# davdwan21/Silent-Speech

Hardware: AMD Instinct MI355X
Metric: clips/sec (30-frame, fwd+bwd) (higher is better)
Workload: dtype f32; 1 GPU; BASELINE config 2: landmark (K=40, D=84) + 64x64 uint8 ROI CNN + 2-layer BiGRU(192), T=30, C=5, train step = fwd + CE(ls .05) + bwd + grad all-reduce + clip(1.0) + Adam, dropout on; batch_per_gpu=256, global_batch=256, frames=30, parallelism=dp1, micro_batches_in_flight=1

## Files before the change

### include/ss_hotpath.h

```cpp
#ifndef SS_HOTPATH_H
#define SS_HOTPATH_H

#include <stdint.h>

#ifdef __cplusplus
extern "C" {
#endif

typedef void* ss_stream_t;

enum ss_status {
  SS_OK = 0,
  SS_ERR_ARG = -1,
  SS_ERR_LAUNCH = -2,
  SS_ERR_UNSUPPORTED = -3
};

int ss_abi_version(void);
const char* ss_status_string(int status);

int ss_feature_fuse(const float* lm, const uint8_t* reset, int B, int T, int K, int w, int h, int a_left,
                    int a_right, int a_up, int a_lo, int variant, float* X, int ldx, float* center,
                    double* fourth, ss_stream_t stream);

// ... 34 lines not shown
int ss_roi_cnn_bwd(const uint8_t* R, int N, int H, int W, int standardize, const float* w1, const float* b1,
                   const float* w2, const float* b2, const float* w3, const float* b3, const float* wfc,
                   const float* bfc, int E, const float* st_a1, const uint8_t* st_i1, const float* st_a2,
                   const uint8_t* st_i2, const uint8_t* st_m3, const float* st_feat, const int* stash_sizes,
                   const float* d_out, int ld_dout, float* g_w1, float* g_b1, float* g_w2, float* g_b2, float* g_w3, float* g_b3,
                   float* g_wfc, float* g_bfc, ss_stream_t stream);

int ss_roi_active_frames(const int32_t* lengths, int B, int T, int* frames, float* emb, int ld_emb, int emb_cols,
                         ss_stream_t stream);
int ss_roi_cnn_fwd_frames(const uint8_t* R, int N, int H, int W, int standardize, const float* w1, const float* b1,
                          const float* w2, const float* b2, const float* w3, const float* b3, const float* wfc,
                          const float* bfc, int E, float* out, int ld_out, float* st_a1, uint8_t* st_i1,
                          float* st_a2, uint8_t* st_i2, uint8_t* st_m3, float* st_feat, const int* stash_sizes,
                          const int* frames, ss_stream_t stream);
int ss_roi_cnn_bwd_frames(const uint8_t* R, int N, int H, int W, int standardize, const float* w1, const float* b1,
                          const float* w2, const float* b2, const float* w3, const float* b3, const float* wfc,
                          const float* bfc, int E, const float* st_a1, const uint8_t* st_i1, const float* st_a2,
                          const uint8_t* st_i2, const uint8_t* st_m3, const float* st_feat, const int* stash_sizes,
                          const float* d_out, int ld_dout, float* g_w1, float* g_b1, float* g_w2, float* g_b2, float* g_w3,
                          float* g_b3, float* g_wfc, float* g_bfc, const int* frames, ss_stream_t stream);

int ss_gemm_f32(int a_kcontig, int b_kcontig, int M, int N, int K, const float* A, int lda, int a_group,
                int a_gstride, int a_off, const float* B, int ldb, int b_group, int b_gstride, int b_off,
                float* C, int ldc, const float* bias, float* a_colsum, int flags, int splits, ss_stream_t stream);

int ss_gemm_f32_batched(int a_kcontig, int b_kcontig, int M, int N, int K, const float* A, int lda, int a_group,
                        int a_gstride, int a_off, const float* B, int ldb, int b_group, int b_gstride, int b_off,
                        float* C, int ldc, const float* bias, float* a_colsum, int flags, int splits, int batch,
                        long stride_a, long stride_b, long stride_c, long stride_bias, long stride_colsum,
                        ss_stream_t stream);

int ss_gemm_splitk_ws_floats(int M, int N, int K, int splits, int batch, long* floats);
int ss_gemm_splitk_reduce(const float* ws, int M, int N, int K, int splits, int batch, float* C, int ldc, long stride_c,
                          ss_stream_t stream);

int ss_train_prologue(float* grads, long n_grads, float* scalars, int n_scalars, int32_t* correct,
                      const int64_t* lengths64, int32_t* lengths32, int B, const float* X, int ld_x, float* Z, int ld_z,
                      int rows, int cols, int* frames, int emb_cols, ss_stream_t stream);

typedef struct ss_gemm_problem {
  int a_kcontig, b_kcontig, M, N, K;
  const float* A;
  int lda, a_group, a_gstride, a_off;
  const float* B;
  int ldb, b_group, b_gstride, b_off;
  float* C;
  int ldc, splits, batch;
  long stride_a, stride_b, stride_c;
} ss_gemm_problem;
int ss_gemm_splitk_group_ws_floats(const ss_gemm_problem* problems, int n, long* floats);
int ss_gemm_f32_splitk_group(const ss_gemm_problem* problems, int n, float* ws, long ws_floats, int flags, ss_stream_t stream);
int ss_gemm_bf16_splitk_group_ws_floats(const ss_gemm_problem* problems, int n, long* floats);
int ss_gemm_bf16_splitk_group(const ss_gemm_problem* problems, int n, float* ws, long ws_floats, ss_stream_t stream);

int ss_zero_f32x2(float* a, long na, float* b, long nb, ss_stream_t stream);

int ss_colsum_f32(const float* A, int rows, int cols, int lda, float* out, ss_stream_t stream);

int ss_batch_gather_f32(const float* src, int D, const int32_t* frame_map, long rows, const float* noise,
                        const int32_t* noise_map, float noise_std, uint64_t seed, float* dst, ss_stream_t stream);
int ss_batch_gather_f32_at(const float* src, int D, const int32_t* frame_map, long rows, const int32_t* noise_map, float noise_std,
                           uint64_t seed, uint64_t noise_first, float* dst, ss_stream_t stream);
int ss_batch_gather_u8(const uint8_t* src, int frame_bytes, const int32_t* frame_map, long rows, uint8_t* dst,
                       ss_stream_t stream);
int ss_epoch_sample(const int32_t* members, int n_members, const int32_t* class_start, int n_classes, uint64_t first, long count,
                    uint64_t seed, int32_t* indices, ss_stream_t stream);
int ss_batch_plan(const int32_t* indices, int B, const int32_t* x_off, const int32_t* x_len, const int32_t* r_off,
                  const int32_t* r_len, const int64_t* y, int n_clips, int max_t, int augment, uint64_t first_row, uint64_t seed,
                  double noise_prob, double drop_prob, int drop_max, int32_t* xmap, int32_t* nmap, int32_t* rmap, int64_t* lens,
                  int64_t* y_out, int32_t* err_flag, ss_stream_t stream);
int ss_batch_plan_aug(const int32_t* indices, int B, const int32_t* x_off, const int32_t* x_len, const int32_t* r_off,
                      const int32_t* r_len, const int64_t* y, int n_clips, int max_t, int augment, uint64_t first_row, uint64_t seed,
                      double noise_prob, double drop_prob, int drop_max, double warp_prob, int warp_lo_pm, int warp_hi_pm,
                      double scale_prob, float scale_lo, float scale_span, double shift_prob, int shift_max_x, int shift_max_y,
                      int32_t* xmap, int32_t* nmap, int32_t* rmap, int64_t* lens, int64_t* y_out, float* row_scale,
                      int32_t* row_shift, int32_t* err_flag, ss_stream_t stream);
int ss_batch_gather_f32_aug(const float* src, int D, const int32_t* frame_map, long rows, const int32_t* noise_map, float noise_std,
                            uint64_t seed, uint64_t noise_first, const float* row_scale, int rows_per_clip, float* dst,
                            ss_stream_t stream);
int ss_batch_gather_u8_shift(const uint8_t* src, int H, int W, const int32_t* frame_map, long rows, const int32_t* row_shift,
                             int rows_per_clip, int shift_max_x, int shift_max_y, uint8_t* dst, ss_stream_t stream);
int ss_batch_gather_z(const float* feat, int D, const int32_t* xmap, const float* emb, int E, const int32_t* rmap,
                      const float* emb_fill, long rows, const int32_t* noise_map, float noise_std, uint64_t seed,
                      uint64_t noise_first, const float* row_scale, int rows_per_clip, float* dst, int ld_dst, ss_stream_t stream);
int ss_batch_plan_mask(int32_t* xmap, int32_t* nmap, int32_t* rmap, const int64_t* lens, int B, int max_t, int D, int H, int W,
                       int augment, uint64_t first_row, uint64_t seed, double time_mask_prob, int time_mask_max,
                       int time_mask_streams, int time_mask_fill, double feat_mask_prob, int feat_mask_max, double cutout_prob,
                       int cut_max_w, int cut_max_h, int cutout_fill, int32_t* row_mask, ss_stream_t stream);
int ss_batch_mask_apply(float* X, int ld_x, int D, uint8_t* R, int H, int W, const int32_t* rmap, const int32_t* row_mask,
                        long rows, int rows_per_clip, int fill, ss_stream_t stream);

int ss_ring_push(float* ring_x, uint8_t* ring_r, int n_streams, int max_t, int D, int frame_bytes,
                 const int32_t* stream_ids, int n, const float* feats, const uint8_t* rois, int32_t* head, int32_t* count,
                 int32_t* frames_seen, ss_stream_t stream);
int ss_ring_tick(const int32_t* stream_ids, int n, int32_t* frames_seen, ss_stream_t stream);
int ss_ring_window_map(const int32_t* stream_ids, int n, int max_t, const int32_t* head, const int32_t* count,
                       int32_t* frame_map, int64_t* lengths, ss_stream_t stream);
int ss_mouth_openness(const float* lm, int n, int K, int mode, int i_top, int i_bot, int i_eye_l, int i_eye_r,
                      double* openness, ss_stream_t stream);
int ss_mouth_gate(const int32_t* stream_ids, int n, const double* openness, double alpha, double open_thr,
                  double close_thr, double* ema, uint8_t* state_open, ss_stream_t stream);
int ss_clip_gate(const int32_t* stream_ids, int n, const double* openv, const uint8_t* face_present, double open_thresh,
                 int start_n, int end_n, int max_clip, int min_clip, int32_t* state, int D, int frame_bytes,
                 const float* feats, const uint8_t* rois, float* clip_x, uint8_t* clip_r, int32_t* append_row,
                 int32_t* emit_len, ss_stream_t stream);

// ... 139 lines not shown
```

### silent_speech_amd/_lib.py

```python
from __future__ import annotations

import ctypes as C
import os

import torch

_HERE = os.path.dirname(os.path.abspath(__file__))
LIB_PATH = os.environ.get("SS_HOTPATH_LIB", os.path.join(_HERE, "libss_hotpath.so"))

_vp = C.c_void_p
_i = C.c_int
_f = C.c_float
_l = C.c_long
_u64 = C.c_uint64
_d = C.c_double

SIGNATURES = {
    "ss_abi_version": [],
    "ss_status_string": [_i],
    "ss_feature_fuse": [_vp, _vp, _i, _i, _i, _i, _i, _i, _i, _i, _i, _i, _vp, _i, _vp, _vp, _vp],
    "ss_feature_fuse_stream": [_vp, _vp, _vp, _i, _i, _i, _i, _i, _i, _i, _i, _i, _i, _d, _d, _vp, _vp, _vp, _i, _vp, _vp, _vp, _vp],
    "ss_roi_norm": [_vp, _i, _i, _i, _vp, _vp, _vp],
    "ss_im2col3x3": [_vp, _i, _i, _i, _i, _vp, _i, _vp],
    "ss_relu_pool2": [_vp, _i, _i, _i, _i, _vp, _vp, _vp],
    "ss_relu_mean": [_vp, _i, _i, _i, _vp, _vp, _vp],
    "ss_mask_scale": [_vp, _vp, _i, _i, _i, _vp, _vp],
    "ss_col2im3x3": [_vp, _i, _i, _i, _i, _i, _vp, _vp],
    "ss_pool2_bwd": [_vp, _vp, _vp, _i, _i, _i, _i, _vp, _vp],
    "ss_roi_crop_idx": [_vp, _vp, _i, _i, _i, _i, _vp, _vp],
    "ss_roi_cnn_fwd": [_vp, _i, _i, _i, _i] + [_vp] * 8 + [_i, _vp, _i, _vp],
    "ss_roi_cnn_fwd_stash": [_vp, _i, _i, _i, _i] + [_vp] * 8 + [_i, _vp, _i] + [_vp] * 6 + [_vp, _vp],
    "ss_roi_cnn_set_max_workgroups": [_i],
    "ss_roi_active_frames": [_vp, _i, _i, _vp, _vp, _i, _i, _vp],
    "ss_roi_cnn_fwd_frames": [_vp, _i, _i, _i, _i] + [_vp] * 8 + [_i, _vp, _i] + [_vp] * 6 + [_vp, _vp, _vp],
    "ss_roi_cnn_bwd_frames": [_vp, _i, _i, _i, _i] + [_vp] * 8 + [_i] + [_vp] * 6 + [_vp, _vp, _i] + [_vp] * 8 + [_vp, _vp],
    "ss_roi_cnn_stash_size": [_i, _i, _vp],
    "ss_roi_cnn_bwd": [_vp, _i, _i, _i, _i] + [_vp] * 8 + [_i] + [_vp] * 6 + [_vp, _vp, _i] + [_vp] * 8 + [_vp],
    "ss_gemm_f32": [_i, _i, _i, _i, _i, _vp, _i, _i, _i, _i, _vp, _i, _i, _i, _i, _vp, _i, _vp, _vp, _i, _i, _vp],
    "ss_gemm_f32_batched": [_i, _i, _i, _i, _i, _vp, _i, _i, _i, _i, _vp, _i, _i, _i, _i, _vp, _i, _vp, _vp, _i, _i, _i,
                            _l, _l, _l, _l, _l, _vp],
    "ss_gemm_bf16_batched": [_i, _i, _i, _i, _i, _vp, _i, _i, _i, _i, _vp, _i, _i, _i, _i, _vp, _i, _vp, _i, _i, _i, _l, _l, _l, _l,
                             _vp],
    "ss_c5_conv1_fwd": [_vp, _i, _i, _vp, _vp, _vp, _vp, _vp, _vp],
    "ss_c5_conv_fwd": [_i, _vp, _i, _vp, _vp, _vp, _vp, _vp],
    "ss_c5_conv_last_fwd": [_vp, _i, _vp, _vp, _vp, _vp, _i, _vp, _i, _vp, _vp, _vp],
    "ss_c5_conv_wgrad": [_i, _vp, _vp, _vp, _i, _vp, _vp, _vp],
    "ss_c5_conv_dgrad": [_i, _vp, _vp, _i, _vp, _vp, _vp],
    "ss_c5_conv_last_wgrad": [_vp, _vp, _i, _i, _vp, _vp, _vp, _i, _vp, _vp, _vp, _vp, _vp],
    "ss_c5_conv_last_dgrad": [_vp, _i, _i, _vp, _vp, _i, _vp, _vp, _vp],
    "ss_c5_conv1_wgrad": [_vp, _i, _i, _vp, _vp, _vp, _vp, _vp, _vp, _vp, _vp],
    "ss_c5_conv2_dgrad_conv1_wgrad": [_vp, _vp, _i, _vp, _vp, _vp, _i, _vp, _vp, _vp, _vp, _vp, _vp],
    "ss_c5_conv12_fwd": [_vp, _i, _i, _vp, _vp, _vp, _vp, _vp, _vp, _vp, _vp],
    "ss_c5_conv_last_fwd_feat": [_vp, _i, _vp, _vp, _vp, _vp, _vp],
    "ss_c5_conv_last_wgrad_df": [_vp, _vp, _vp, _i, _vp, _vp, _vp, _l, _vp],
    "ss_c5_conv_wgrad_ws": [_i, _vp, _vp, _vp, _i, _vp, _vp, _vp, _l, _vp],
    "ss_c5_conv2_wgrad_rc_ws": [_vp, _vp, _i, _vp, _vp, _vp, _vp, _i, _vp, _vp, _vp, _l, _vp],
    "ss_c5_conv_last_dgrad_df": [_vp, _vp, _i, _vp, _vp, _vp],
    "ss_c5_conv12_fwd_i1": [_vp, _i, _i, _vp, _vp, _vp, _vp, _vp, _vp, _vp, _vp, _vp],
    "ss_c5_conv2_dgrad_conv1_wgrad_i1": [_vp, _vp, _i, _vp, _vp, _vp, _i, _vp, _vp, _vp, _vp, _vp, _vp, _vp],
    "ss_c5_conv2_wgrad_rc": [_vp, _vp, _i, _vp, _vp, _vp, _vp, _i, _vp, _vp, _vp],
    "ss_gru_bf16_prep": [_vp, _vp, _i, _vp, _vp, _vp, _vp, _i, _vp, _vp],
    "ss_gru_bf16_ws_bytes": [_i, _i, _vp],
    "ss_gru_bf16_sync_bytes": [_i, _i, _i, _vp],
    "ss_gru_bf16_fwd": [_vp, _vp, _vp, _vp, _vp, _i, _i, _i, _vp, _vp, _vp, _vp, _f, _u64, _u64, _vp, _vp, _l, _vp],
    "ss_gru_bf16_bwd": [_vp, _vp, _vp, _vp, _vp, _i, _i, _i, _vp, _vp, _f, _u64, _u64, _vp, _vp, _vp, _vp, _vp, _vp, _l, _vp],
    "ss_cvt_bf16_rows": [_vp, _i, _vp, _i, _l, _i, _f, _u64, _u64, _vp],
    "ss_gemm_splitk_ws_floats": [_i, _i, _i, _i, _i, _vp],
    "ss_gemm_splitk_reduce": [_vp, _i, _i, _i, _i, _i, _vp, _i, _l, _vp],
    "ss_gemm_splitk_group_ws_floats": [_vp, _i, _vp],
    "ss_gemm_f32_splitk_group": [_vp, _i, _vp, _l, _i, _vp],
    "ss_gemm_bf16_splitk_group_ws_floats": [_vp, _i, _vp],
    "ss_gemm_bf16_splitk_group": [_vp, _i, _vp, _l, _vp],
    "ss_colsum_f32": [_vp, _i, _i, _i, _vp, _vp],
    "ss_zero_f32x2": [_vp, _l, _vp, _l, _vp],
    "ss_train_prologue": [_vp, _l, _vp, _i, _vp, _vp, _vp, _i, _vp, _i, _vp, _i, _i, _i, _vp, _i, _vp],
    "ss_batch_gather_f32": [_vp, _i, _vp, _l, _vp, _vp, _f, _u64, _vp, _vp],
    "ss_batch_gather_f32_at": [_vp, _i, _vp, _l, _vp, _f, _u64, _u64, _vp, _vp],
    "ss_batch_gather_u8": [_vp, _i, _vp, _l, _vp, _vp],
    "ss_epoch_sample": [_vp, _i, _vp, _i, _u64, _l, _u64, _vp, _vp],
    "ss_batch_plan": [_vp, _i, _vp, _vp, _vp, _vp, _vp, _i, _i, _i, _u64, _u64, _d, _d, _i, _vp, _vp, _vp, _vp, _vp, _vp, _vp],
    "ss_batch_plan_aug": [_vp, _i, _vp, _vp, _vp, _vp, _vp, _i, _i, _i, _u64, _u64, _d, _d, _i, _d, _i, _i, _d, _f, _f, _d, _i, _i,
                          _vp, _vp, _vp, _vp, _vp, _vp, _vp, _vp, _vp],
    "ss_batch_gather_f32_aug": [_vp, _i, _vp, _l, _vp, _f, _u64, _u64, _vp, _i, _vp, _vp],
    "ss_batch_gather_u8_shift": [_vp, _i, _i, _vp, _l, _vp, _i, _i, _i, _vp, _vp],
    "ss_batch_gather_z": [_vp, _i, _vp, _vp, _i, _vp, _vp, _l, _vp, _f, _u64, _u64, _vp, _i, _vp, _i, _vp],
    "ss_batch_plan_mask": [_vp, _vp, _vp, _vp, _i, _i, _i, _i, _i, _i, _u64, _u64, _d, _i, _i, _i, _d, _i, _d, _i, _i, _i, _vp, _vp],
    "ss_batch_mask_apply": [_vp, _i, _i, _vp, _i, _i, _vp, _vp, _l, _i, _i, _vp],
    "ss_crop_gray_resize": [_vp, _i, _i, _i, _vp, _i, _i, _i, _vp, _vp],
    "ss_ring_tick": [_vp, _i, _vp, _vp],
    "ss_ring_push": [_vp, _vp, _i, _i, _i, _i, _vp, _i, _vp, _vp, _vp, _vp, _vp, _vp],
    "ss_ring_window_map": [_vp, _i, _i, _vp, _vp, _vp, _vp, _vp],
    "ss_mouth_openness": [_vp, _i, _i, _i, _i, _i, _i, _i, _vp, _vp],
    "ss_mouth_gate": [_vp, _i, _vp, _d, _d, _d, _vp, _vp, _vp],
    "ss_clip_gate": [_vp, _i, _vp, _vp, _d, _i, _i, _i, _i, _vp, _i, _i, _vp, _vp, _vp, _vp, _vp, _vp, _vp],
    "ss_gru_fwd": [_vp, _vp, _vp, _vp, _vp, _vp, _i, _i, _i, _vp, _vp, _vp, _vp],
    "ss_gru_fwd_drop": [_vp, _vp, _vp, _vp, _vp, _vp, _i, _i, _i, _vp, _vp, _vp, _f, _u64, _u64, _vp, _vp],
    "ss_gru_sync_bytes": [_i, _i, _i, _vp],
    "ss_gru_bwd": [_vp, _vp, _vp, _vp, _vp, _vp, _i, _i, _i, _vp, _f, _u64, _u64, _vp, _vp, _vp, _vp, _vp, _vp],
    "ss_gru_bias_grad": [_vp, _i, _i, _vp, _vp, _vp, _vp, _vp],
    "ss_attn_pool_fwd": [_vp, _vp, _vp, _vp, _i, _i, _i, _vp, _vp, _vp],
    "ss_attn_pool_bwd": [_vp, _vp, _vp, _vp, _vp, _i, _i, _i, _vp, _vp, _vp, _vp],
    "ss_tail_fwd": [_vp] * 11 + [_i] * 5 + [_f, _f, _u64, _u64, _f, _f] + [_vp] * 10 + [_vp],
    "ss_tail_fwd_w": [_vp] * 11 + [_i] * 5 + [_f, _f, _u64, _u64, _f, _vp, _vp] + [_vp] * 10 + [_vp],
    "ss_tail_bwd": [_vp] * 11 + [_i] * 5 + [_f, _u64, _u64] + [_vp] * 7 + [_vp],
    "ss_layernorm_fwd": [_vp, _vp, _vp, _i, _i, _f, _vp, _vp, _vp, _vp],
    "ss_layernorm_bwd": [_vp, _vp, _vp, _vp, _i, _i, _vp, _vp, _vp, _vp],
    "ss_dropout": [_vp, _vp, _l, _f, _u64, _u64, _vp, _vp],
    "ss_ce_ls_fwd_bwd": [_vp, _vp, _i, _i, _f, _f, _vp, _vp, _vp, _vp],
    "ss_eval_accum": [_vp, _vp, _i, _i, _f, _i, _vp, _vp, _vp, _vp, _vp, _vp, _vp, _vp],
    "ss_ce_ls_w_fwd_bwd": [_vp, _vp, _i, _i, _f, _vp, _vp, _vp, _vp, _vp, _vp],
    "ss_class_weight_sum": [_vp, _l, _vp, _i, _vp, _vp],
    "ss_eval_accum_w": [_vp, _vp, _i, _i, _f, _i, _vp, _vp, _vp, _vp, _vp, _vp, _vp, _vp, _vp, _vp],
    "ss_softmax_topk": [_vp, _i, _i, _i, _vp, _vp, _vp],
    "ss_sumsq_f32": [_vp, _l, _vp, _vp],
    "ss_adam_clip": [_vp, _vp, _vp, _vp, _l, _vp, _f, _f, _f, _f, _f, _f, _i, _vp],
    "ss_adam_clip_ema": [_vp, _vp, _vp, _vp, _vp, _l, _vp, _f, _f, _f, _f, _f, _f, _i, _f, _vp],
    "ss_swap_f32": [_vp, _vp, _l, _vp],
    "ss_copy_rows_f32": [_vp, _i, _vp, _i, _i, _i, _vp],
}
_RESTYPES = {"ss_status_string": C.c_char_p}

_lib = None


def load():
# ... 106 lines not shown
```

### silent_speech_amd/csrc/gemm.hip

```cpp
#include <stdlib.h>

#include <type_traits>

#define SS_STAMP_ROW ((int)(blockIdx.x + gridDim.x * (blockIdx.y + gridDim.y * blockIdx.z)))
#include "ss_common.h"

STAMP_TABLE(ss_debug_stamps_gemm)

namespace {

constexpr int BM = 128, BN = 64, BK = 16;
constexpr int LDK = BK + 4;
constexpr int LDM_A = BM + 4;
constexpr int LDM_B = BN + 4;

struct RowMap {
  int G, S, off;
  __device__ __forceinline__ long operator()(int r) const {
    if (G == 0x7fffffff) return r + off;
    return (long)(r / G) * S + (r % G) + off;
  }
};

struct GemmParams {
// ... 808 lines not shown
    for (int mt = 0; mt < 3; ++mt) a[mt] = *reinterpret_cast<const f32x4*>(st + offA[mt]);
#pragma unroll
    for (int nt = 0; nt < 6; ++nt) b[nt] = *reinterpret_cast<const f32x4*>(st + offB[nt]);
  };
  auto mma = [&]() {
#pragma unroll
    for (int kk = 0; kk < 4; ++kk)
#pragma unroll
      for (int mt = 0; mt < 3; ++mt)
#pragma unroll
        for (int nt = 0; nt < 6; ++nt) acc[mt][nt] = mfma16(a[mt][kk], b[nt][kk], acc[mt][nt]);
  };
  ring_k_loop<W_LPW>(
      nfull, rem, issue,
      [&](int stage, int refill) {
        if (refill >= 0) issue(refill);
        read(dlds + stage * W_STAGE);
        mma();
      },
      [&](int kvalid) { dp.tail(dlds, kvalid); });
  constexpr int LDS_C = 96 + 4;
  static_assert(WT * LDS_C <= DSTAGES * W_STAGE, "half an output tile is staged in the k-tile ring");
  float* Cb = P.C + bi * P.sC;
  const float* bias = P.bias ? P.bias + bi * P.sBias : nullptr;
  const bool vec_ok = (P.ldc & 3) == 0 && (reinterpret_cast<uintptr_t>(Cb) & 15) == 0;
#pragma unroll 1
  for (int h = 0; h < 2; ++h) {
    __syncthreads();
    if (wn == h) {
#pragma unroll
      for (int mt = 0; mt < 3; ++mt)
#pragma unroll
        for (int nt = 0; nt < 6; ++nt) {
          const int col = nt * 16 + i, gc = n0 + h * 96 + col;
          const float bv = (bias && gc < P.N) ? bias[gc] : 0.f;
#pragma unroll
          for (int r = 0; r < 4; ++r) dlds[(wm * 48 + mt * 16 + 4 * g + r) * LDS_C + col] = acc[mt][nt][r] + bv;
        }
    }
    __syncthreads();
    for (int q = threadIdx.x; q < WT * 24; q += WNT) {
      const int row = q / 24, c4 = 4 * (q % 24);
      const int gr = m0 + row, gc = n0 + h * 96 + c4;
      if (gr < P.M && gc < P.N) {
        const f32x4 v = *reinterpret_cast<const f32x4*>(&dlds[row * LDS_C + c4]);
        float* dst = Cb + (long)gr * P.ldc + gc;
        if (vec_ok && gc + 4 <= P.N) *reinterpret_cast<f32x4*>(dst) = v;
        else
          for (int e = 0; e < 4; ++e)
            if (gc + e < P.N) dst[e] = v[e];
      }
    }
  }
}
}

int splitk_slices(int K, int splits, int* per_out) {
  const int per = ceil_div(ceil_div(K, splits), BK * KSUB) * BK * KSUB;
  if (per_out) *per_out = per;
  return ceil_div(K, per);
}

long splitk_slab_floats(int M, int N, int K, int splits, int batch) {
  return (long)batch * splitk_slices(K, splits, nullptr) * ceil_div(M, BM) * ceil_div(N, BN) * BM * BN;
}

bool al16(const void* q) { return (reinterpret_cast<uintptr_t>(q) & 15) == 0; }

constexpr size_t dma_lds = (size_t)DSTAGES * D_STAGE * sizeof(float);
constexpr size_t wide_lds = (size_t)DSTAGES * wide::W_STAGE * sizeof(float);

template <class F>
void by_layout(bool a_kcontig, bool b_kcontig, F&& f) {
  using T = std::true_type;
  using N = std::false_type;
  if (a_kcontig && b_kcontig) f(T{}, T{});
  else if (a_kcontig && !b_kcontig) f(T{}, N{});
  else if (!a_kcontig && b_kcontig) f(N{}, T{});
  else f(N{}, N{});
}

}

extern "C" int ss_gemm_splitk_ws_floats(int M, int N, int K, int splits, int batch, long* floats) {
  SS_REQUIRE(M > 0 && N > 0 && K > 0 && splits >= 1 && batch >= 1 && floats, SS_ERR_ARG);
  *floats = splitk_slab_floats(M, N, K, splits, batch);
  return SS_OK;
}

extern "C" int ss_gemm_splitk_reduce(const float* ws, int M, int N, int K, int splits, int batch, float* C, int ldc,
                                     long stride_c, ss_stream_t stream) {
  SS_REQUIRE(ws && C && M > 0 && N > 0 && K > 0 && splits >= 1 && batch >= 1 && ldc >= N, SS_ERR_ARG);
  SS_REQUIRE((reinterpret_cast<uintptr_t>(ws) & 15) == 0, SS_ERR_ARG);
  const int nz = splitk_slices(K, splits, nullptr), gx = ceil_div(N, BN), gy = ceil_div(M, BM);
  const ReduceItem r{reinterpret_cast<const f32x4*>(ws), nz, gx, gy, M, N, C, ldc, stride_c};
  hipLaunchKernelGGL(splitk_reduce_kernel, dim3((unsigned)(batch * gx * gy * 8)), dim3(256), 0, static_cast<hipStream_t>(stream), r);
  return ss_launch_status();
}

struct GemmExtras {
  const float* bias;
  float* a_colsum;
  int flags;
  long stride_bias, stride_colsum;
};
struct GemmLaunch {
// ... 188 lines not shown
    }
  }
  GemmGroup gg;
  ReduceGroup rg;
  gg.n = rg.n = n;
  gg.first[0] = rg.first[0] = 0;
  bool grouped = true;
  for (int j = 0; j < n; ++j) {
    const ss_gemm_problem& q = problems[j];
    const ss_gemm_problem slab = group_slab_gemm(problems, j, ws);
    GemmLaunch gl;
    const int st = gemm_prepare(slab, kSlabGemm, &gl);
    if (st != SS_OK) return st;
    SS_REQUIRE(q.C && q.ldc >= q.N, SS_ERR_ARG);
    grouped = grouped && gl.dma_ok && q.a_kcontig == problems[0].a_kcontig && q.b_kcontig == problems[0].b_kcontig;
    gg.p[j] = gl.p;
    gg.gx[j] = gl.grid.x; gg.gy[j] = gl.grid.y;
    gg.first[j + 1] = gg.first[j] + (int)(gl.grid.x * gl.grid.y * gl.grid.z);
    rg.it[j] = ReduceItem{reinterpret_cast<const f32x4*>(slab.C), gl.p.nz, (int)gl.grid.x, (int)gl.grid.y, q.M, q.N, q.C, q.ldc, q.stride_c};
    rg.first[j + 1] = rg.first[j] + (int)(q.batch * gl.grid.x * gl.grid.y * 8);
  }
  for (int j = n; j < GEMM_GROUP_MAX; ++j) {
    gg.p[j] = gg.p[0]; gg.gx[j] = gg.gy[j] = 1; gg.first[j + 1] = gg.first[n];
    rg.it[j] = rg.it[0]; rg.first[j + 1] = rg.first[n];
  }
  hipStream_t s = static_cast<hipStream_t>(stream);
  if (!grouped) {
    for (int j = 0; j < n; ++j) {
      const ss_gemm_problem& q = problems[j];
      const ss_gemm_problem slab = group_slab_gemm(problems, j, ws);
      int st = gemm_batched(slab, kSlabGemm, stream);
      if (st != SS_OK) return st;
      st = ss_gemm_splitk_reduce(slab.C, q.M, q.N, q.K, q.splits, q.batch, q.C, q.ldc, q.stride_c, stream);
      if (st != SS_OK) return st;
    }
    return SS_OK;
  }
  const dim3 ggrid((unsigned)gg.first[n]), block(256);
  by_layout(problems[0].a_kcontig, problems[0].b_kcontig, [&](auto a, auto b) {
    hipLaunchKernelGGL((gemm_dma_group_kernel<decltype(a)::value, decltype(b)::value>), ggrid, block, dma_lds, s, gg);
  });
  if (ss_launch_status() != SS_OK) return SS_ERR_LAUNCH;
  hipLaunchKernelGGL(splitk_reduce_group_kernel, dim3((unsigned)rg.first[n]), dim3(256), 0, s, rg);
  return ss_launch_status();
}

extern "C" int ss_gemm_f32(int a_kcontig, int b_kcontig, int M, int N, int K, const float* A, int lda, int a_group,
                           int a_gstride, int a_off, const float* B, int ldb, int b_group, int b_gstride, int b_off,
                           float* C, int ldc, const float* bias, float* a_colsum, int flags, int splits,
                           ss_stream_t stream) {
  return ss_gemm_f32_batched(a_kcontig, b_kcontig, M, N, K, A, lda, a_group, a_gstride, a_off, B, ldb, b_group,
                             b_gstride, b_off, C, ldc, bias, a_colsum, flags, splits, 1, 0, 0, 0, 0, 0, stream);
}
```

### silent_speech_amd/engine.py

```python
from __future__ import annotations

import os

from dataclasses import dataclass
from typing import Dict, Optional

import torch

from . import _lib as L

INT_MAX = 2**31 - 1
_HH_TARGET = 512
USE_SIDE_STREAM = True


@dataclass
class Config:
    x_dim: int
    num_classes: int
    use_roi: bool
    roi_emb: int = 32
    hidden: int = 192
    gru_layers: int = 2
    roi_standardize: bool = True
    gru_dropout: float = 0.1
    head_dropout: float = 0.2
    head_mid: int = 128
    ln_eps: float = 1e-5
    cnn_channels: tuple = (8, 16, 24)
    precision: str = "f32"

    @property
    def in_dim(self) -> int:
        return self.x_dim + (self.roi_emb if self.use_roi else 0)


def gemm(a_kc, b_kc, M, N, K, A, lda, B, ldb, Cm, ldc, bias=None, accumulate=False, relu=False, splits=1,
         a_map=(INT_MAX, 0, 0), b_map=(INT_MAX, 0, 0), a_colsum=None, tag="gemm", batch=1, strides=(0, 0, 0, 0, 0),
         atomic=False, splitk_ws: Optional[torch.Tensor] = None, sum_batch=False):
    if splitk_ws is not None and splits > 1 and accumulate and not relu and bias is None:
        need = L.gemm_splitk_ws_floats(M, N, K, splits, batch)
        if splitk_ws.numel() < need:
            raise RuntimeError(f"split-K workspace too small: {splitk_ws.numel()} < {need}")
        L.call("ss_gemm_f32_batched", int(a_kc), int(b_kc), M, N, K, A, lda, a_map[0], a_map[1], a_map[2], B, ldb,
               b_map[0], b_map[1], b_map[2], splitk_ws.data_ptr(), N, None, a_colsum, 8, splits, batch,
               strides[0], strides[1], 0, 0, strides[4], L.stream(), tag=tag)
        L.call("ss_gemm_splitk_reduce", splitk_ws.data_ptr(), M, N, K, splits, batch, Cm, ldc, strides[2], L.stream(),
               tag=tag + "_reduce")
        return
    flags = (1 if accumulate else 0) | (2 if relu else 0) | (4 if atomic else 0) | (16 if sum_batch else 0)
    L.call("ss_gemm_f32_batched", int(a_kc), int(b_kc), M, N, K, A, lda, a_map[0], a_map[1], a_map[2], B, ldb,
           b_map[0], b_map[1], b_map[2], Cm, ldc, bias, a_colsum, flags, splits, batch, *strides, L.stream(), tag=tag)


_SPLITK_TARGET = 768
DW_WIDE_ALONE = 1
SKIP_PADDED_FRAMES = os.environ.get("SS_CNN_SKIP_PADDING", "1") != "0"

_DX_SPLIT_CAP = 2


def split_k(M, N, K, batch=1, target_wgs=_SPLITK_TARGET):
    tiles = -(-M // 128) * -(-N // 64) * batch
    return max(1, min(K // 128, target_wgs // tiles))


def dw_shapes(cfg, B, T, l):
    H, N = cfg.hidden, B * T
    K = cfg.in_dim if l == 0 else 2 * H
    out = [(3 * H, K, N, split_k(3 * H, K, N, 2))]
    if T > 1:
        Kh = B * (T - 1)
        out += [(2 * H, H, Kh, split_k(2 * H, H, Kh, 2, _HH_TARGET)), (H, H, Kh, split_k(H, H, Kh, 2, _HH_TARGET))]
    return out


def dw_records(cfg, B, T, l, esize, ld_in, dg, lin, hp, g_ih, g_hh, splits=None):
    H, N = cfg.hidden, B * T
    shapes = dw_shapes(cfg, B, T, l)
    splits = splits or [sh[3] for sh in shapes]
    K = shapes[0][1]

    def rec(shape, A, a_map, B_, ldb, b_map, Cm, ldc, sp, sa, sb, sc):
        return L.GemmProblem(0, 0, *shape[:3], A, 4 * H, *a_map, B_, ldb, *b_map, Cm, ldc, sp, 2, sa, sb, sc)

    ident = (INT_MAX, 0, 0)
    out = [rec(shapes[0], dg, ident, lin, ld_in, ident, g_ih[0], K, splits[0], N * 4 * H, 0, g_ih[1])]
    if T > 1:
        am, bm = (T - 1, T, 1), (T - 1, T, 0)
        sa, sb = N * 4 * H - 4 * H, H + 2 * H
        out.append(rec(shapes[1], dg, am, hp, 2 * H, bm, g_hh[0], H, splits[1], sa, sb, g_hh[1]))
        out.append(rec(shapes[2], dg + 3 * H * esize, am, hp, 2 * H, bm, g_hh[0] + 2 * H * H * 4, H, splits[2], sa, sb, g_hh[1]))
    return out


def dw_problems(ws, G, cfg, l, lin, ld_in):
    wi, wir = f"gru.weight_ih_l{l}", f"gru.weight_ih_l{l}_reverse"
    wh, whr = f"gru.weight_hh_l{l}", f"gru.weight_hh_l{l}_reverse"
    return dw_records(cfg, ws.B, ws.T, l, 4, ld_in, ws.dG[l].data_ptr(), lin, ws.out[l].data_ptr(),
                      (G[wi].data_ptr(), _pstride(G, wi, wir)), (G[wh].data_ptr(), _pstride(G, wh, whr)))


def _pstride(P, a: str, b: str) -> int:
    return (P[b].data_ptr() - P[a].data_ptr()) // 4


def _addr(t: torch.Tensor, offset_elems: int = 0) -> int:
    return t.data_ptr() + offset_elems * t.element_size()


def zero_buffers(bufs) -> None:
    bufs = [b for b in bufs if b is not None and b.numel()]
    for k in range(0, len(bufs), 2):
        a, b = bufs[k], bufs[k + 1] if k + 1 < len(bufs) else None
        L.call("ss_zero_f32x2", a.data_ptr(), a.numel(), L.ptr(b), b.numel() if b is not None else 0, L.stream())


def check_gru_sync(ws) -> None:
    sync = getattr(ws, "gru_sync", None)
    if sync is not None and int(sync[2]) != 0:
        raise RuntimeError(f"multi-CU GRU recurrence: {int(sync[2])} exchange waits timed out (a partner workgroup never "
                           "arrived); results since then are poisoned with NaN")


_SIDE_STREAMS: Dict[tuple, "torch.cuda.Stream"] = {}


def side_stream(device, slot=0) -> "torch.cuda.Stream":
    dev = torch.device(device)
    key = (dev.index if dev.index is not None else torch.cuda.current_device(), slot if isinstance(slot, int) else 0)
    st = _SIDE_STREAMS.get(key)
    if st is None:
        st = _SIDE_STREAMS[key] = torch.cuda.Stream(device=dev, priority=torch.cuda.Stream.priority_range()[0])
    return st


def make_workspace(cfg: Config, B: int, T: int, roi_hw, device, train: bool, slot=0):
    if cfg.precision == "bf16":
        from .engine_bf16 import WorkspaceBf16

        return WorkspaceBf16(cfg, B, T, roi_hw, device, train, slot)
    return Workspace(cfg, B, T, roi_hw, device, train, slot)


class WorkspaceBase:

    def __init__(self, cfg: Config, B: int, T: int, roi_hw, device, train: bool, slot=0):
        self.cfg, self.B, self.T, self.roi_hw, self.train = cfg, B, T, roi_hw, train
        self.stash_gen, self.stash_live = 0, False
        N, H = B * T, cfg.hidden
        f32 = dict(device=device, dtype=torch.float32)
        self.lengths = torch.empty(B, device=device, dtype=torch.int32)
        self.side = side_stream(device, slot) if train else None
        self.ev_fork = torch.cuda.Event() if train else None
        self.ev_join = torch.cuda.Event() if train else None
        self.ev_cnn_fwd = torch.cuda.Event() if train else None
        self.ev_zero = torch.cuda.Event() if train else None
        self.stagger = False
        self.Z = torch.empty(N, cfg.in_dim, **f32) if cfg.use_roi and roi_hw is not None else None
        self.frames = self.frames_seen = None
        self.gi = [torch.empty(2, N, 3 * H, **f32) for _ in range(cfg.gru_layers)]
        self.out = [torch.empty(N, 2 * H, **f32) for _ in range(cfg.gru_layers)]
        self.attn = torch.empty(B, T, **f32)
        self.ln = torch.empty(B, 2 * H, **f32)
        self.mid = torch.empty(B, cfg.head_mid, **f32)
        self.mid_drop = torch.empty(B, cfg.head_mid, **f32)
        self.logits = torch.empty(B, cfg.num_classes, **f32)
        if train:
            self.save = [torch.empty(2, N, 4, H, **f32) for _ in range(cfg.gru_layers)]
            self.d_out = torch.empty(N, 2 * H, **f32)
            self.d_lower = [None] + [torch.empty(N, 2 * H, **f32) for _ in range(1, cfg.gru_layers)]
            self.xhat = torch.empty(B, 2 * H, **f32)
            self.rstd = torch.empty(B, **f32)
            self.d_logits = torch.empty(B, cfg.num_classes, **f32)
            self.d_mid = torch.empty(B, cfg.head_mid, **f32)
            self.tail_part = torch.empty(B, 3, 2 * H, **f32)
            self.dZ = torch.empty(N, cfg.in_dim, **f32) if cfg.use_roi and roi_hw is not None else None


class Workspace(WorkspaceBase):

    bf16 = False

    def __init__(self, cfg: Config, B: int, T: int, roi_hw, device, train: bool, slot=0):
        super().__init__(cfg, B, T, roi_hw, device, train, slot)
        N, H = B * T, cfg.hidden
        f32 = dict(device=device, dtype=torch.float32)
        u8 = dict(device=device, dtype=torch.uint8)
        nb = L.gru_sync_bytes(B, T, H)
        self.gru_sync = torch.zeros(nb // 4, device=device, dtype=torch.int32) if nb else None
        self.cnn_generic = None
        if cfg.use_roi and roi_hw is not None:
            from . import cnn_generic

            if not cnn_generic.fused_supported(*roi_hw):
                self.cnn_generic = cnn_generic.GenericCnn(N, roi_hw[0], roi_hw[1], device, train)
        self.out_drop = [torch.empty(N, 2 * H, **f32) for _ in range(cfg.gru_layers - 1)]
        if train:
            self.dG = [torch.empty(2, N, 4, H, **f32) for _ in range(cfg.gru_layers)]
            self.splitk_ws = torch.empty(max(L.gemm_group_ws_floats(dw_records(cfg, B, T, l, 4, 0, 0, 0, 0, (0, 0), (0, 0)))
                                             for l in range(cfg.gru_layers)), **f32)
            if cfg.use_roi and roi_hw is not None and self.cnn_generic is None:
                Hh, Ww = roi_hw
                self.cnn_sizes = L.cnn_stash_sizes(Hh, Ww)
                n_a1, n_a2, n_i1, n_i2, n_m3, n_feat = self.cnn_sizes
                self.st_a1 = torch.empty(N, n_a1, **f32)
                self.st_i1 = torch.empty(N, n_i1, **u8)
                self.st_a2 = torch.empty(N, n_a2, **f32)
                self.st_i2 = torch.empty(N, n_i2, **u8)
                self.st_m3 = torch.empty(N, n_m3, **u8)
                self.st_feat = torch.empty(N, n_feat, **f32)
        if cfg.use_roi and roi_hw is not None and self.cnn_generic is None and SKIP_PADDED_FRAMES:
            self.frames = torch.empty(1 + N, device=device, dtype=torch.int32)
        if self.frames is not None and train:
            self.frames_seen = torch.full((1,), -1, dtype=torch.int32).pin_memory()
        self.walk_listed = self.frames is not None


CNN_PARAMS = ("roi_cnn.net.0.weight", "roi_cnn.net.0.bias", "roi_cnn.net.3.weight", "roi_cnn.net.3.bias",
              "roi_cnn.net.6.weight", "roi_cnn.net.6.bias", "roi_cnn.fc.weight", "roi_cnn.fc.bias")


def tail_fwd(P, cfg: Config, ws, top, train, stash, seed, ce):
    p_drop = cfg.head_dropout if train else 0.0
    y_ptr, ls, denom, loss_ptr, correct_ptr, cw_ptr, den_ptr = (tuple(ce) + (None, None))[:7] if ce is not None else (None, 0.0, 1.0, None, None, None, None)
    name, ce_norm = ("ss_tail_fwd_w", (cw_ptr, den_ptr)) if cw_ptr else ("ss_tail_fwd", (denom,))
    L.call(name, top.data_ptr(), ws.lengths.data_ptr(), P["pool.score.weight"].data_ptr(),
           P["pool.score.bias"].data_ptr(), P["head.0.weight"].data_ptr(), P["head.0.bias"].data_ptr(),
           P["head.1.weight"].data_ptr(), P["head.1.bias"].data_ptr(), P["head.4.weight"].data_ptr(),
           P["head.4.bias"].data_ptr(), y_ptr, ws.B, ws.T, 2 * cfg.hidden, cfg.head_mid, cfg.num_classes, cfg.ln_eps, p_drop, seed,
           7 << 40, ls, *ce_norm, ws.attn.data_ptr() if stash else None, ws.xhat.data_ptr() if stash else None,
           ws.rstd.data_ptr() if stash else None, ws.ln.data_ptr() if stash else None,
           ws.mid.data_ptr() if stash else None, ws.mid_drop.data_ptr() if stash else None, ws.logits.data_ptr(),
           ws.d_logits.data_ptr() if ce is not None else None, loss_ptr, correct_ptr, L.stream())
    return ws.logits


def tail_bwd(P, G, cfg: Config, ws, d_logits, train, seed):
    L.call("ss_tail_bwd", ws.out[-1].data_ptr(), ws.lengths.data_ptr(), P["pool.score.weight"].data_ptr(),
           P["head.0.weight"].data_ptr(), P["head.1.weight"].data_ptr(), P["head.4.weight"].data_ptr(),
           ws.attn.data_ptr(), ws.xhat.data_ptr(), ws.rstd.data_ptr(), ws.mid.data_ptr(), d_logits.data_ptr(), ws.B, ws.T,
           2 * cfg.hidden, cfg.head_mid, cfg.num_classes, cfg.head_dropout if train else 0.0, seed, 7 << 40, ws.d_mid.data_ptr(),
           ws.d_out.data_ptr(), G["head.0.weight"].data_ptr(), G["head.0.bias"].data_ptr(), G["pool.score.weight"].data_ptr(),
           G["pool.score.bias"].data_ptr(), ws.tail_part.data_ptr(), L.stream())


def head_grads(G, cfg: Config, ws, d_logits):
    B, H, C, MID = ws.B, cfg.hidden, cfg.num_classes, cfg.head_mid
    zero_buffers(ws.d_lower[1:] + ([ws.dZ] if cfg.use_roi else []))
    ws.ev_zero.record()
    if ws.frames_seen is not None:
        ws.frames_seen.copy_(ws.frames[:1], non_blocking=True)
    for k_, name_ in enumerate(("head.0.weight", "head.0.bias", "pool.score.weight")):
        L.call("ss_colsum_f32", _addr(ws.tail_part, k_ * 2 * H), B, 2 * H, 3 * 2 * H, G[name_].data_ptr(), L.stream())
    gemm(0, 0, C, MID, B, d_logits.data_ptr(), C, ws.mid_drop.data_ptr(), MID, G["head.4.weight"].data_ptr(), MID,
         accumulate=True, atomic=True, a_colsum=G["head.4.bias"].data_ptr())
    gemm(0, 0, MID, 2 * H, B, ws.d_mid.data_ptr(), MID, ws.ln.data_ptr(), 2 * H, G["head.1.weight"].data_ptr(),
         2 * H, accumulate=True, atomic=True, a_colsum=G["head.1.bias"].data_ptr())


def fork(ws, on: bool) -> None:
    if on:
        ws.ev_fork.record()


def on_side(ws, on: bool, work) -> None:
    if not on:
        return work()
    with torch.cuda.stream(ws.side):
        ws.side.wait_event(ws.ev_fork)
        work()


def join_side(ws, on: bool) -> None:
    if on:
        ws.ev_join.record(ws.side)
        torch.cuda.current_stream().wait_event(ws.ev_join)


def forward(P: Dict[str, torch.Tensor], cfg: Config, ws: Workspace, X: torch.Tensor, R: Optional[torch.Tensor], *,
            train: bool, stash: bool = False, seed: int = 0, ce=None, x_in_place: bool = False, z_ready: bool = False) -> torch.Tensor:
    if ws.bf16:
        from . import engine_bf16

        if z_ready:
            raise RuntimeError("z_ready: the bf16 engine has no path for rows that already hold the embeddings")
        return engine_bf16.forward(P, cfg, ws, X, R, train=train, stash=stash, seed=seed, ce=ce, x_in_place=x_in_place)
    B, T, H, N = ws.B, ws.T, cfg.hidden, ws.B * ws.T
    s = L.stream()
    if stash and not ws.train:
        raise RuntimeError("stash=True needs a training workspace")
    if z_ready:
        if not cfg.use_roi or X.shape[2] != cfg.in_dim:
            raise RuntimeError("z_ready: rows of width in_dim = x_dim + roi_emb of a use_roi model")
        if (stash or train) and ws.roi_hw is not None:
            raise RuntimeError("z_ready: train / stash need a workspace built with roi_hw=None")
        layer_in, ld_in = X.data_ptr(), cfg.in_dim
    elif cfg.use_roi:
        Hh, Ww = ws.roi_hw
        ws_Z = ws.Z
        if not x_in_place:
            L.call("ss_copy_rows_f32", X.data_ptr(), cfg.x_dim, ws_Z.data_ptr(), cfg.in_dim, N, cfg.x_dim, s)
        if ws.cnn_generic is not None:
# ... 39 lines not shown

def backward(P: Dict[str, torch.Tensor], G: Dict[str, torch.Tensor], cfg: Config, ws: Workspace, X: torch.Tensor,
             R: Optional[torch.Tensor], d_logits: torch.Tensor, *, train: bool, seed: int = 0,
             d_X: Optional[torch.Tensor] = None, frozen_cnn: bool = False) -> None:
    if frozen_cnn and (ws.bf16 or not cfg.use_roi or ws.roi_hw is not None or d_X is not None):
        raise RuntimeError("frozen_cnn: the f32 engine, a use_roi model, a workspace built with roi_hw=None, and no d_X")
    if ws.bf16:
        from . import engine_bf16

        return engine_bf16.backward(P, G, cfg, ws, X, R, d_logits, train=train, seed=seed, d_X=d_X)
    B, T, H, N = ws.B, ws.T, cfg.hidden, ws.B * ws.T
    s = L.stream()
    tail_bwd(P, G, cfg, ws, d_logits, train, seed)
    fork(ws, USE_SIDE_STREAM)
    use_drop = train and cfg.gru_dropout > 0.0
    zero_waited = False
    for l in range(cfg.gru_layers - 1, -1, -1):
        K = cfg.in_dim if l == 0 else 2 * H
        top_layer = l == cfg.gru_layers - 1
        g_in = ws.d_out if top_layer else ws.d_lower[l + 1]
        L.call("ss_gru_bwd", g_in.data_ptr(), ws.out[l].data_ptr(), ws.save[l].data_ptr(),
               P[f"gru.weight_hh_l{l}"].data_ptr(), P[f"gru.weight_hh_l{l}_reverse"].data_ptr(),
               ws.lengths.data_ptr(), B, T, H, ws.dG[l].data_ptr(),
               0.0 if (top_layer or not use_drop) else cfg.gru_dropout, seed, (l + 1) << 40,
               G[f"gru.bias_ih_l{l}"].data_ptr(), G[f"gru.bias_hh_l{l}"].data_ptr(),
               G[f"gru.bias_ih_l{l}_reverse"].data_ptr(), G[f"gru.bias_hh_l{l}_reverse"].data_ptr(), L.ptr(ws.gru_sync), s)
        if top_layer:
            on_side(ws, USE_SIDE_STREAM, lambda: head_grads(G, cfg, ws, d_logits))
        if l == 0:
            if frozen_cnn:
                lin, ld_in = X.data_ptr(), cfg.in_dim
            elif cfg.use_roi:
                lin, ld_in = ws.Z.data_ptr(), cfg.in_dim
            else:
                lin, ld_in = X.data_ptr(), cfg.x_dim
        else:
            use_drop = train and cfg.gru_dropout > 0.0
            lin, ld_in = (ws.out_drop[l - 1] if use_drop else ws.out[l - 1]).data_ptr(), 2 * H
        def side_work(l=l, lin=lin, ld_in=ld_in):
            fork(ws, USE_SIDE_STREAM)
            on_side(ws, USE_SIDE_STREAM, lambda: L.call(
                "ss_gemm_f32_splitk_group", *L.gemm_group(dw_problems(ws, G, cfg, l, lin, ld_in)), ws.splitk_ws.data_ptr(),
                ws.splitk_ws.numel(), DW_WIDE_ALONE if l == 0 else 0, L.stream(), tag="gemm_gru_dW"))
        if l == 0:
            side_work()
        need_dx = (l > 0) or (cfg.use_roi and not frozen_cnn) or (d_X is not None)
        if need_dx:
            if l > 0:
                dst, ld_dst = ws.d_lower[l].data_ptr(), 2 * H
            elif cfg.use_roi:
                dst, ld_dst = ws.dZ.data_ptr(), cfg.in_dim
            else:
                dst, ld_dst = d_X.data_ptr(), cfg.x_dim
                zero_buffers([d_X])
            if USE_SIDE_STREAM and not zero_waited:
                torch.cuda.current_stream().wait_event(ws.ev_zero)
                zero_waited = True
            wi, wir = f"gru.weight_ih_l{l}", f"gru.weight_ih_l{l}_reverse"
            c0 = cfg.x_dim if (l == 0 and cfg.use_roi and d_X is None) else 0
            tiles = -(-N // 128) * -(-(K - c0) // 64) * 2
            dx_splits = max(1, min(_DX_SPLIT_CAP, 768 // tiles, (3 * H) // 96))
            gemm(1, 0, N, K - c0, 3 * H, ws.dG[l].data_ptr(), 4 * H, _addr(P[wi], c0), K, dst + 4 * c0, ld_dst,
                 accumulate=True, atomic=True, tag="gemm_gru_dX", batch=2, splits=dx_splits,
                 strides=(N * 4 * H, _pstride(P, wi, wir), 0, 0, 0))
        if l > 0:
            side_work()
    if cfg.use_roi and d_X is not None:
        L.call("ss_copy_rows_f32", ws.dZ.data_ptr(), cfg.in_dim, d_X.data_ptr(), cfg.x_dim, N, cfg.x_dim, s)
    join_side(ws, USE_SIDE_STREAM)
    if cfg.use_roi and not frozen_cnn:
        Hh, Ww = ws.roi_hw
        if ws.cnn_generic is not None:
            ws.cnn_generic.backward(P, G, cfg.roi_emb, _addr(ws.dZ, cfg.x_dim), cfg.in_dim)
        else:
            L.call("ss_roi_cnn_bwd_frames", R.data_ptr(), N, Hh, Ww, int(cfg.roi_standardize), *[P[k].data_ptr() for k in CNN_PARAMS],
                   cfg.roi_emb, ws.st_a1.data_ptr(), ws.st_i1.data_ptr(), ws.st_a2.data_ptr(), ws.st_i2.data_ptr(),
                   ws.st_m3.data_ptr(), ws.st_feat.data_ptr(), ws.cnn_sizes.ptr, _addr(ws.dZ, cfg.x_dim), cfg.in_dim,
                   *[G[k].data_ptr() for k in CNN_PARAMS], L.ptr(ws.frames) if ws.walk_listed else None, s, tag="ss_roi_cnn_bwd")
```

Baseline: 133,300 clips/s.

## Add dedicated GRU input-gradient kernel summing both directions without atomics or zeroing

```diff
diff --git a/include/ss_hotpath.h b/include/ss_hotpath.h
--- a/include/ss_hotpath.h
+++ b/include/ss_hotpath.h
@@ -110,6 +110,9 @@
 int ss_gemm_f32_splitk_group(const ss_gemm_problem* problems, int n, float* ws, long ws_floats, int flags, ss_stream_t stream);
 int ss_gemm_bf16_splitk_group_ws_floats(const ss_gemm_problem* problems, int n, long* floats);
 int ss_gemm_bf16_splitk_group(const ss_gemm_problem* problems, int n, float* ws, long ws_floats, ss_stream_t stream);
+
+int ss_gru_dx_f32(int M, int N, int K, const float* A, int lda, long stride_a, const float* B, int ldb, int b_col0,
+                  long stride_b, float* C, int ldc, ss_stream_t stream);
 
 int ss_zero_f32x2(float* a, long na, float* b, long nb, ss_stream_t stream);
 
diff --git a/silent_speech_amd/_lib.py b/silent_speech_amd/_lib.py
--- a/silent_speech_amd/_lib.py
+++ b/silent_speech_amd/_lib.py
@@ -71,6 +71,7 @@
     "ss_gemm_f32_splitk_group": [_vp, _i, _vp, _l, _i, _vp],
     "ss_gemm_bf16_splitk_group_ws_floats": [_vp, _i, _vp],
     "ss_gemm_bf16_splitk_group": [_vp, _i, _vp, _l, _vp],
+    "ss_gru_dx_f32": [_i, _i, _i, _vp, _i, _l, _vp, _i, _i, _l, _vp, _i, _vp],
     "ss_colsum_f32": [_vp, _i, _i, _i, _vp, _vp],
     "ss_zero_f32x2": [_vp, _l, _vp, _l, _vp],
     "ss_train_prologue": [_vp, _l, _vp, _i, _vp, _vp, _vp, _i, _vp, _i, _vp, _i, _i, _i, _vp, _i, _vp],
diff --git a/silent_speech_amd/csrc/gemm.hip b/silent_speech_amd/csrc/gemm.hip
--- a/silent_speech_amd/csrc/gemm.hip
+++ b/silent_speech_amd/csrc/gemm.hip
@@ -884,6 +884,187 @@
       }
     }
   }
+}
+}
+
+namespace dx {
+constexpr int XCDS = 8;
+struct DxParams {
+  const float *A, *B;
+  float* C;
+  int M, N, K, lda, ldb, ldc, gx, gy;
+  long sA, sB;
+  int dma;
+};
+
+template <int TM_, int TN_, int WGM_, int WGN_>
+struct Tile {
+  static constexpr int TM = TM_, TN = TN_, WGM = WGM_, WGN = WGN_;
+  static constexpr int NW = WGM * WGN, NT = 64 * NW;
+  static constexpr int WTM = TM / WGM, WTN = TN / WGN, MT = WTM / 16, NTL = WTN / 16;
+  static constexpr int PA = TM / 16, PB = TN / 16;
+  static constexpr int LPW = (PA + PB) / NW;
+  static constexpr int STAGE = (TM + TN) * BK;
+  static constexpr size_t LDS = (size_t)DSTAGES * STAGE * sizeof(float);
+  static_assert((PA + PB) % NW == 0, "pieces deal evenly over the waves");
+  static_assert(TM * (TN + 4) <= DSTAGES * STAGE, "the output tile is staged in the k-tile ring");
+  static_assert(WTM % 16 == 0 && WTN % 16 == 0 && TN % 4 == 0, "whole MFMA tiles per wave");
+};
+using Wide = Tile<64, 192, 2, 4>;
+using Narrow = Tile<32, 32, 2, 2>;
+
+template <class T>
+struct Pieces {
+  const float* src[T::LPW];
+  long step[T::LPW];
+  static __device__ __forceinline__ int piece(int n) { return (threadIdx.x >> 6) + T::NW * n; }
+  static __device__ __forceinline__ bool isb(int n) { return piece(n) >= T::PA; }
+  static __device__ __forceinline__ int slot(int n) { return (piece(n) - (isb(n) ? T::PA : 0)) * 64 + (threadIdx.x & 63); }
+  __device__ __forceinline__ void init(const DxParams& P, int dir, int m0, int n0) {
+#pragma unroll
+    for (int n = 0; n < T::LPW; ++n) {
+      const int sl = slot(n);
+      if (isb(n)) {
+        src[n] = P.B + dir * P.sB + (long)KRowImage<T::TN>::k(sl) * P.ldb + KRowImage<T::TN>::src_col(sl, n0, P.N);
+        step[n] = (long)BK * P.ldb;
+      } else {
+        src[n] = P.A + dir * P.sA + (long)KcImage::src_row(sl, m0, P.M) * P.lda + KcImage::src_k(sl);
+        step[n] = BK;
+      }
+    }
+  }
+  __device__ __forceinline__ void issue(unsigned stage_byte) const {
+#pragma unroll
+    for (int n = 0; n < T::LPW; ++n) ss_dma16(src[n], stage_byte + piece(n) * 1024);
+  }
+  __device__ __forceinline__ void advance() {
+#pragma unroll
+    for (int n = 0; n < T::LPW; ++n) src[n] += step[n];
+  }
+  static __device__ __forceinline__ void stage(float* img, const DxParams& P, int dir, int m0, int n0, int k0) {
+#pragma unroll
+    for (int n = 0; n < T::LPW; ++n) {
+      const int sl = slot(n);
+      f32x4 v = {0.f, 0.f, 0.f, 0.f};
+      if (isb(n)) {
+        const int k = k0 + KRowImage<T::TN>::k(sl), col = n0 + 4 * KRowImage<T::TN>::src_unit(sl);
+        if (k < P.K) {
+          const float* s = P.B + dir * P.sB + (long)k * P.ldb + col;
+#pragma unroll
+          for (int e = 0; e < 4; ++e)
+            if (col + e < P.N) v[e] = s[e];
+        }
+      } else {
+        const int kq = k0 + KcImage::src_k(sl);
+        const float* s = P.A + dir * P.sA + (long)KcImage::src_row(sl, m0, P.M) * P.lda + kq;
+#pragma unroll
+        for (int e = 0; e < 4; ++e)
+          if (kq + e < P.K) v[e] = s[e];
+      }
+      *reinterpret_cast<f32x4*>(img + piece(n) * 256 + 4 * (threadIdx.x & 63)) = v;
+    }
+  }
+};
+
+template <class T>
+__global__ __launch_bounds__(T::NT) void gru_dx_kernel(DxParams P) {
+  extern __shared__ __attribute__((aligned(16))) float dlds[];
+  const int per = XCDS * P.gx, grp = blockIdx.x / per, r = blockIdx.x - grp * per;
+  const int by = grp * XCDS + r % XCDS, bx = r / XCDS;
+  if (by >= P.gy) return;
+  const int m0 = by * T::TM, n0 = bx * T::TN;
+  const int nfull = P.K / BK, rem = P.K - nfull * BK;
+  const int lane = threadIdx.x & 63, wid = threadIdx.x >> 6;
+  const int wm = wid / T::WGN, wn = wid % T::WGN, i = lane & 15, g = lane >> 4;
+  int offA[T::MT], offB[T::NTL];
+#pragma unroll
+  for (int mt = 0; mt < T::MT; ++mt) offA[mt] = KcImage::frag(wm * T::WTM + mt * 16 + i, g);
+#pragma unroll
+  for (int nt = 0; nt < T::NTL; ++nt) offB[nt] = T::TM * BK + KRowImage<T::TN>::frag(wn * T::WTN + nt * 16 + i, g);
+  f32x4 acc[T::MT][T::NTL];
+#pragma unroll
+  for (int mt = 0; mt < T::MT; ++mt)
+#pragma unroll
+    for (int nt = 0; nt < T::NTL; ++nt) acc[mt][nt] = f32x4{0.f, 0.f, 0.f, 0.f};
+  auto multiply = [&](const float* st) {
+    f32x4 a[T::MT];
+    float b[T::NTL][4];
+#pragma unroll
+    for (int mt = 0; mt < T::MT; ++mt) a[mt] = *reinterpret_cast<const f32x4*>(st + offA[mt]);
+#pragma unroll
+    for (int kk = 0; kk < 4; ++kk)
+#pragma unroll
+      for (int nt = 0; nt < T::NTL; ++nt) b[nt][kk] = st[offB[nt] + kk * T::TN];
+#pragma unroll
+    for (int kk = 0; kk < 4; ++kk)
+#pragma unroll
+      for (int mt = 0; mt < T::MT; ++mt)
+#pragma unroll
+        for (int nt = 0; nt < T::NTL; ++nt) acc[mt][nt] = mfma16(a[mt][kk], b[nt][kk], acc[mt][nt]);
+  };
+  if (P.dma) {
+    Pieces<T> dp;
+    const int passes = rem ? 2 : 1;
+    for (int pass = 0; pass < passes; ++pass) {
+      if (pass) __syncthreads();
+      dp.init(P, pass, m0, n0);
+      int issued = 0;
+      auto issue = [&](int buf) {
+        dp.issue((unsigned)(buf * T::STAGE * 4));
+        dp.advance();
+        if (++issued == nfull && !rem) dp.init(P, 1, m0, n0);
+      };
+      ring_k_loop<T::LPW>(
+          rem ? nfull : 2 * nfull, rem, issue,
+          [&](int stage, int refill) {
+            if (refill >= 0) issue(refill);
+            multiply(dlds + stage * T::STAGE);
+          },
+          [&](int) { Pieces<T>::stage(dlds, P, pass, m0, n0, nfull * BK); });
+    }
+  } else {
+    for (int dir = 0; dir < 2; ++dir)
+      for (int k0 = 0; k0 < P.K; k0 += BK) {
+        __syncthreads();
+        Pieces<T>::stage(dlds, P, dir, m0, n0, k0);
+        __syncthreads();
+        multiply(dlds);
+      }
+  }
+  constexpr int LDS_C = T::TN + 4, Q = T::TN / 4;
+  __syncthreads();
+#pragma unroll
+  for (int mt = 0; mt < T::MT; ++mt)
+#pragma unroll
+    for (int nt = 0; nt < T::NTL; ++nt)
+#pragma unroll
+      for (int rr = 0; rr < 4; ++rr)
+        dlds[(wm * T::WTM + mt * 16 + 4 * g + rr) * LDS_C + wn * T::WTN + nt * 16 + i] = acc[mt][nt][rr];
+  __syncthreads();
+  const bool vec_ok = (P.ldc & 3) == 0 && (reinterpret_cast<uintptr_t>(P.C) & 15) == 0;
+  for (int q = threadIdx.x; q < T::TM * Q; q += T::NT) {
+    const int row = q / Q, c4 = 4 * (q % Q);
+    const int gr = m0 + row, gc = n0 + c4;
+    if (gr < P.M && gc < P.N) {
+      const f32x4 v = *reinterpret_cast<const f32x4*>(&dlds[row * LDS_C + c4]);
+      float* dst = P.C + (long)gr * P.ldc + gc;
+      if (vec_ok && gc + 4 <= P.N) *reinterpret_cast<f32x4*>(dst) = v;
+      else
+        for (int e = 0; e < 4; ++e)
+          if (gc + e < P.N) dst[e] = v[e];
+    }
+  }
+}
+
+template <class T>
+int launch(DxParams P, hipStream_t s) {
+  P.gx = ceil_div(P.N, T::TN);
+  P.gy = ceil_div(P.M, T::TM);
+  const long grid = (long)ceil_div(P.gy, XCDS) * XCDS * P.gx;
+  SS_REQUIRE(grid <= 0x7fffffff, SS_ERR_UNSUPPORTED);
+  SS_REQUIRE(ss_dynamic_lds(reinterpret_cast<const void*>(gru_dx_kernel<T>), (int)T::LDS) == SS_OK, SS_ERR_LAUNCH);
+  hipLaunchKernelGGL(gru_dx_kernel<T>, dim3((unsigned)grid), dim3(T::NT), T::LDS, s, P);
+  return ss_launch_status();
 }
 }
 
@@ -1178,3 +1359,17 @@
   return ss_gemm_f32_batched(a_kcontig, b_kcontig, M, N, K, A, lda, a_group, a_gstride, a_off, B, ldb, b_group,
                              b_gstride, b_off, C, ldc, bias, a_colsum, flags, splits, 1, 0, 0, 0, 0, 0, stream);
 }
+
+extern "C" int ss_gru_dx_f32(int M, int N, int K, const float* A, int lda, long stride_a, const float* B, int ldb, int b_col0,
+                             long stride_b, float* C, int ldc, ss_stream_t stream) {
+  SS_REQUIRE(M > 0 && N > 0 && K > 0 && A && B && C, SS_ERR_ARG);
+  SS_REQUIRE(lda >= K && b_col0 >= 0 && (long)b_col0 + N <= ldb && ldc >= N, SS_ERR_ARG);
+  dx::DxParams P;
+  P.A = A; P.B = B + b_col0; P.C = C;
+  P.M = M; P.N = N; P.K = K; P.lda = lda; P.ldb = ldb; P.ldc = ldc;
+  P.sA = stride_a; P.sB = stride_b;
+  P.dma = al16(P.A) && al16(P.B) && (lda & 3) == 0 && (ldb & 3) == 0 && (stride_a & 3) == 0 && (stride_b & 3) == 0 && N >= 4 &&
+          (N & 3) == 0;
+  hipStream_t s = static_cast<hipStream_t>(stream);
+  return N <= dx::Narrow::TN ? dx::launch<dx::Narrow>(P, s) : dx::launch<dx::Wide>(P, s);
+}
diff --git a/silent_speech_amd/engine.py b/silent_speech_amd/engine.py
--- a/silent_speech_amd/engine.py
+++ b/silent_speech_amd/engine.py
@@ -58,6 +58,12 @@
 SKIP_PADDED_FRAMES = os.environ.get("SS_CNN_SKIP_PADDING", "1") != "0"
 
 _DX_SPLIT_CAP = 2
+DX_ONE_LAUNCH_MIN_FILL = 0.8
+
+
+def dx_one_launch(cfg, rows: int, device) -> bool:
+    cus = torch.cuda.get_device_properties(device).multi_processor_count
+    return -(-rows // 64) * -(-2 * cfg.hidden // 192) >= DX_ONE_LAUNCH_MIN_FILL * cus
 
 
 def split_k(M, N, K, batch=1, target_wgs=_SPLITK_TARGET):
@@ -156,6 +162,7 @@
         self.ev_join = torch.cuda.Event() if train else None
         self.ev_cnn_fwd = torch.cuda.Event() if train else None
         self.ev_zero = torch.cuda.Event() if train else None
+        self.dx_one_launch = False
         self.stagger = False
         self.Z = torch.empty(N, cfg.in_dim, **f32) if cfg.use_roi and roi_hw is not None else None
         self.frames = self.frames_seen = None
@@ -188,6 +195,7 @@
         f32 = dict(device=device, dtype=torch.float32)
         u8 = dict(device=device, dtype=torch.uint8)
         nb = L.gru_sync_bytes(B, T, H)
+        self.dx_one_launch = train and dx_one_launch(cfg, N, device)
         self.gru_sync = torch.zeros(nb // 4, device=device, dtype=torch.int32) if nb else None
         self.cnn_generic = None
         if cfg.use_roi and roi_hw is not None:
@@ -247,8 +255,9 @@
 
 def head_grads(G, cfg: Config, ws, d_logits):
     B, H, C, MID = ws.B, cfg.hidden, cfg.num_classes, cfg.head_mid
-    zero_buffers(ws.d_lower[1:] + ([ws.dZ] if cfg.use_roi else []))
-    ws.ev_zero.record()
+    if not ws.dx_one_launch:
+        zero_buffers(ws.d_lower[1:] + ([ws.dZ] if cfg.use_roi else []))
+        ws.ev_zero.record()
     if ws.frames_seen is not None:
         ws.frames_seen.copy_(ws.frames[:1], non_blocking=True)
     for k_, name_ in enumerate(("head.0.weight", "head.0.bias", "pool.score.weight")):
@@ -394,17 +403,22 @@
                 dst, ld_dst = ws.dZ.data_ptr(), cfg.in_dim
             else:
                 dst, ld_dst = d_X.data_ptr(), cfg.x_dim
-                zero_buffers([d_X])
-            if USE_SIDE_STREAM and not zero_waited:
-                torch.cuda.current_stream().wait_event(ws.ev_zero)
-                zero_waited = True
             wi, wir = f"gru.weight_ih_l{l}", f"gru.weight_ih_l{l}_reverse"
             c0 = cfg.x_dim if (l == 0 and cfg.use_roi and d_X is None) else 0
-            tiles = -(-N // 128) * -(-(K - c0) // 64) * 2
-            dx_splits = max(1, min(_DX_SPLIT_CAP, 768 // tiles, (3 * H) // 96))
-            gemm(1, 0, N, K - c0, 3 * H, ws.dG[l].data_ptr(), 4 * H, _addr(P[wi], c0), K, dst + 4 * c0, ld_dst,
-                 accumulate=True, atomic=True, tag="gemm_gru_dX", batch=2, splits=dx_splits,
-                 strides=(N * 4 * H, _pstride(P, wi, wir), 0, 0, 0))
+            if ws.dx_one_launch:
+                L.call("ss_gru_dx_f32", N, K - c0, 3 * H, ws.dG[l].data_ptr(), 4 * H, N * 4 * H, P[wi].data_ptr(), K, c0,
+                       _pstride(P, wi, wir), dst + 4 * c0, ld_dst, s, tag="gemm_gru_dX")
+            else:
+                if l == 0 and not cfg.use_roi:
+                    zero_buffers([d_X])
+                if USE_SIDE_STREAM and not zero_waited:
+                    torch.cuda.current_stream().wait_event(ws.ev_zero)
+                    zero_waited = True
+                tiles = -(-N // 128) * -(-(K - c0) // 64) * 2
+                dx_splits = max(1, min(_DX_SPLIT_CAP, 768 // tiles, (3 * H) // 96))
+                gemm(1, 0, N, K - c0, 3 * H, ws.dG[l].data_ptr(), 4 * H, _addr(P[wi], c0), K, dst + 4 * c0, ld_dst,
+                     accumulate=True, atomic=True, tag="gemm_gru_dX", batch=2, splits=dx_splits,
+                     strides=(N * 4 * H, _pstride(P, wi, wir), 0, 0, 0))
         if l > 0:
             side_work()
     if cfg.use_roi and d_X is not None:
```

After: 134,800 clips/s, median of 6. 1.01x the previous value.
